# montekki/thaler-study

Hardware: AMD Instinct MI355X
Metric: field mul-adds/sec in sumcheck prover, n=28 vars (higher is better)
Workload: dtype u64

## Files before the change

### thaler-study_amd/csrc/kernels.hpp

```cpp
#pragma once
#include <hip/hip_runtime.h>

#include <type_traits>

#include "field.hpp"

namespace sc {

constexpr int kBlock = 256;
constexpr int kWave = 64;
constexpr int kMaxSums = 27;

typedef unsigned long long ull2 __attribute__((ext_vector_type(2)));

template <bool NT>
__device__ __forceinline__ ull2 ld16(const ull2* __restrict__ p) {
  if constexpr (NT) return __builtin_nontemporal_load(p);
  else return *p;
}
template <bool NT>
__device__ __forceinline__ void st16(ull2* __restrict__ p, ull2 v) {
  if constexpr (NT) __builtin_nontemporal_store(v, p);
  else *p = v;
}

struct FoldW {
  u64 w[16];
};

template <class F, int KF, int IN>
__device__ __forceinline__ void fold_run(const F& f, u64 (&v)[IN], const FoldW& fw) {
  if constexpr (KF == 1) {
    const u64 r0 = fw.w[1];
#pragma unroll
    for (int b = 0; b < IN / 2; ++b) v[b] = f.add(v[2 * b], f.mul(r0, f.sub(v[2 * b + 1], v[2 * b])));
  } else if constexpr (KF >= 2) {
    constexpr int G = 1 << KF;
#pragma unroll
    for (int b = 0; b < IN / G; ++b) {
      typename F::Acc3 acc;
      f.acc3_zero(acc);
#pragma unroll
      for (int c = 0; c < G; ++c) f.acc3_mac(acc, v[G * b + c], fw.w[c]);
      v[b] = f.acc3_get(acc);
    }
  }
}

template <class F>
__device__ __forceinline__ void extend_quads(const F& f, const X64 (&ta)[4], const X64 (&tb)[4], X64 (&ea)[3][3],
                                             X64 (&eb)[3][3]) {
  const X64 ha[4] = {ta[1], ta[3], ta[2], ta[3]}, la[4] = {ta[0], ta[2], ta[0], ta[1]};
  const X64 hb[4] = {tb[1], tb[3], tb[2], tb[3]}, lb[4] = {tb[0], tb[2], tb[0], tb[1]};
  X64 da[4], db[4];
  f.sub4(da, ha, la);
  f.sub4(db, hb, lb);
  const X64 ch[2] = {da[1], db[1]}, cl[2] = {da[0], db[0]};
  X64 corner[2];
  f.sub2(corner, ch, cl);
  ea[0][0] = ta[0]; ea[1][0] = ta[1]; ea[2][0] = da[0];
  ea[0][1] = ta[2]; ea[1][1] = ta[3]; ea[2][1] = da[1];
  ea[0][2] = da[2]; ea[1][2] = da[3]; ea[2][2] = corner[0];
  eb[0][0] = tb[0]; eb[1][0] = tb[1]; eb[2][0] = db[0];
  eb[0][1] = tb[2]; eb[1][1] = tb[3]; eb[2][1] = db[1];
  eb[0][2] = db[2]; eb[1][2] = db[3]; eb[2][2] = corner[1];
}

template <class F, int KS>
__device__ __forceinline__ void accumulate_run(const F& f, typename F::Acc* acc, const u64* a,
                                               const u64* b) {
  if constexpr (KS == 1) {
    f.acc_mac(acc[0], a[0], b[0]);
    f.acc_mac(acc[1], a[1], b[1]);
    f.acc_mac(acc[2], f.sub(a[1], a[0]), f.sub(b[1], b[0]));
  } else if constexpr (KS == 2) {
    X64 ea[3][3], eb[3][3];
    const X64 ta[4] = {split64(a[0]), split64(a[1]), split64(a[2]), split64(a[3])};
    const X64 tb[4] = {split64(b[0]), split64(b[1]), split64(b[2]), split64(b[3])};
    extend_quads(f, ta, tb, ea, eb);
#pragma unroll
    for (int u = 0; u < 3; ++u)
#pragma unroll
      for (int v = 0; v < 3; ++v) f.acc_mac(acc[3 * u + v], ea[u][v], eb[u][v]);
  }
}

template <class F>
__device__ __forceinline__ void accumulate_octet(const F& f, typename F::Acc* acc, const u64* a, const u64* b) {
#pragma unroll
  for (int step = 0; step < 3; ++step) {
    const int w = (step == 0) ? 0 : (step == 1) ? 2 : 1;
    X64 sa[4], sb[4];
    if (w == 2) {
      const X64 ah[4] = {split64(a[4]), split64(a[5]), split64(a[6]), split64(a[7])};
      const X64 al[4] = {split64(a[0]), split64(a[1]), split64(a[2]), split64(a[3])};
      const X64 bh[4] = {split64(b[4]), split64(b[5]), split64(b[6]), split64(b[7])};
      const X64 bl[4] = {split64(b[0]), split64(b[1]), split64(b[2]), split64(b[3])};
      f.sub4(sa, ah, al);
      f.sub4(sb, bh, bl);
    } else {
#pragma unroll
      for (int i = 0; i < 4; ++i) {
        sa[i] = split64(a[4 * w + i]);
        sb[i] = split64(b[4 * w + i]);
      }
    }
    X64 ea[3][3], eb[3][3];
    extend_quads(f, sa, sb, ea, eb);
#pragma unroll
    for (int u = 0; u < 3; ++u)
#pragma unroll
      for (int v = 0; v < 3; ++v) f.acc_mac(acc[(3 * u + v) * 3 + w], ea[u][v], eb[u][v]);
  }
}

__device__ __forceinline__ u64 shfl_down_u64(u64 v, int off) {
  return (u64)__shfl_down((unsigned long long)v, off, kWave);
}
__device__ __forceinline__ u64 shfl_u64(u64 v, int src) {
  return (u64)__shfl((unsigned long long)v, src, kWave);
}

template <class F, int NS>
__device__ __forceinline__ void block_reduce(const F& f, u64 (&res)[NS], u64* lds ) {
#pragma unroll
  for (int off = kWave / 2; off >= 1; off >>= 1) {
#pragma unroll
    for (int s = 0; s < NS; ++s) res[s] = f.add(res[s], shfl_down_u64(res[s], off));
  }
  const int lane = threadIdx.x & (kWave - 1), wave = threadIdx.x / kWave;
  if (lane == 0) {
#pragma unroll
    for (int s = 0; s < NS; ++s) lds[wave * NS + s] = res[s];
  }
  __syncthreads();
  if (threadIdx.x < NS) {
    u64 t = lds[threadIdx.x];
    const int n_waves = (int)blockDim.x / kWave;
    for (int w = 1; w < n_waves; ++w) t = f.add(t, lds[w * NS + threadIdx.x]);
    res[0] = t;
  }
}

__device__ __forceinline__ void write_split(u64* out, int s, u64 v) {
  out[2 * s] = v & 0xFFFFFFFFull;
  out[2 * s + 1] = v >> 32;
}

template <int NP>
__device__ __forceinline__ int swz_slot(int q) {
  if constexpr (NP == 1) return q;
  static_assert(NP == 2 || NP == 4 || NP == 8 || NP == 16, "pieces per lane");
  constexpr int SH = (NP == 2) ? 3 : (NP == 4) ? 2 : (NP == 8) ? 1 : 0;
  const int l = q / NP;
  return (q & ~(NP - 1)) | ((q ^ (l >> SH)) & (NP - 1));
}
__device__ __forceinline__ void wave_lds_sync() {
  asm volatile("s_waitcnt lgkmcnt(0)" ::: "memory");
  __builtin_amdgcn_wave_barrier();
}
template <int NP>
__device__ __forceinline__ void transpose_to_runs(ull2* __restrict__ lds, ull2 (&v)[NP], int lane) {
  if constexpr (NP > 1) {
#pragma unroll
    for (int k = 0; k < NP; ++k) lds[swz_slot<NP>(64 * k + lane)] = v[k];
    wave_lds_sync();
#pragma unroll
    for (int m = 0; m < NP; ++m) v[m] = lds[swz_slot<NP>(NP * lane + m)];
    wave_lds_sync();
  }
}
template <int NP>
__device__ __forceinline__ void transpose_to_pieces(ull2* __restrict__ lds, ull2 (&v)[NP], int lane) {
  if constexpr (NP > 1) {
#pragma unroll
    for (int m = 0; m < NP; ++m) lds[swz_slot<NP>(NP * lane + m)] = v[m];
    wave_lds_sync();
#pragma unroll
    for (int k = 0; k < NP; ++k) v[k] = lds[swz_slot<NP>(64 * k + lane)];
    wave_lds_sync();
  }
}

}

#include "kernels/pass.hpp"
#include "kernels/grid_pass.hpp"
#include "kernels/gram.hpp"
#include "kernels/mle.hpp"
#include "kernels/gkr.hpp"
#include "kernels/circuit.hpp"
#include "kernels/triangle.hpp"
#include "kernels/matmul.hpp"
#include "kernels/batch.hpp"
#include "kernels/sha256.hpp"
#include "kernels/merkle.hpp"
#include "kernels/pcs.hpp"
#include "kernels/row_code.hpp"
#include "kernels/ligero.hpp"
#include "kernels/ligero_long.hpp"
#include "kernels/rs_fold.hpp"
#include "kernels/expander.hpp"
#include "kernels/expander_long.hpp"
#include "kernels/peer.hpp"
#include "kernels/r1cs.hpp"
```

### thaler-study_amd/csrc/kernels/batch.hpp

```cpp
#pragma once

namespace sc {

constexpr int kBatchMaxBlocks = 128;
struct BatchDesc {
  const u64* a;
  const u64* b;
  u64* a2;
  u64* b2;
  GridW gw;
};
struct BatchOut {
  u64* partials;
  unsigned* tickets;
  u64* cells;
  u64* mailbox;
  u64 seq;
  int host_out;
};

template <class F, int KS>
__device__ __forceinline__ void batch_finish(const F& f, u64 total, const BatchOut& out, int inst) {
  constexpr int kPow3[6] = {1, 3, 9, 27, 81, 243};
  constexpr int cells = kPow3[KS], kLoads = 16;
  __shared__ int lds_flag;
  const int tid = threadIdx.x, n_blocks = gridDim.x;
  const u64* rows = out.partials + (size_t)inst * n_blocks * kGridChunk;
  if (tid < cells)
    __hip_atomic_store(out.partials + ((size_t)inst * n_blocks + blockIdx.x) * kGridChunk + tid, total, __ATOMIC_RELAXED,
                       __HIP_MEMORY_SCOPE_AGENT);
  asm volatile("s_waitcnt vmcnt(0)" ::: "memory");
  __syncthreads();
  if (tid == 0) {
    const unsigned t = __hip_atomic_fetch_add(out.tickets + 1 + inst, 1u, __ATOMIC_RELAXED, __HIP_MEMORY_SCOPE_AGENT);
    const int last = (t == (unsigned)n_blocks - 1) ? 1 : 0;
    if (last) {
      __builtin_amdgcn_fence(__ATOMIC_ACQUIRE, "agent");
      asm volatile("s_waitcnt vmcnt(0)" ::: "memory");
    }
    lds_flag = last;
  }
  __syncthreads();
  if (!lds_flag) return;
  if (tid < cells) {
    u64 s = 0;
    for (int q0 = 0; q0 < n_blocks; q0 += kLoads) {
      u64 x[kLoads];
#pragma unroll
      for (int q = 0; q < kLoads; ++q)
        x[q] = (q0 + q < n_blocks) ? __hip_atomic_load(rows + (size_t)(q0 + q) * kGridChunk + tid, __ATOMIC_RELAXED, __HIP_MEMORY_SCOPE_AGENT) : 0;
#pragma unroll
      for (int q = 0; q < kLoads; ++q) s = f.add(s, x[q]);
    }
    __hip_atomic_store(out.cells + (size_t)inst * kGridMaxCells + tid, s, __ATOMIC_RELAXED, __HIP_MEMORY_SCOPE_SYSTEM);
  }
  if (tid == 0) __hip_atomic_store(out.tickets + 1 + inst, 0u, __ATOMIC_RELAXED, __HIP_MEMORY_SCOPE_AGENT);
  asm volatile("s_waitcnt vmcnt(0)" ::: "memory");
  __syncthreads();
  if (tid == 0) {
    const unsigned t = __hip_atomic_fetch_add(out.tickets, 1u, __ATOMIC_RELAXED, __HIP_MEMORY_SCOPE_AGENT);
    if (t == gridDim.y - 1) {
      __builtin_amdgcn_fence(__ATOMIC_ACQUIRE, "agent");
      __hip_atomic_store(out.tickets, 0u, __ATOMIC_RELAXED, __HIP_MEMORY_SCOPE_AGENT);
      __hip_atomic_store(out.mailbox + kMailboxSeq, out.seq, __ATOMIC_RELEASE, __HIP_MEMORY_SCOPE_SYSTEM);
    }
  }
}

template <class F, int KS, bool PF>
__global__ void __launch_bounds__(kBlock)
batch_pass_kernel(F f, const BatchDesc* __restrict__ desc, int kf, size_t n_out, BatchOut out) {
  const int inst = blockIdx.y;
  const BatchDesc& d = desc[inst];
  const GridW gw = d.gw;
  const u64 total = wgrid_body<F, KS, PF>(f, d.a, d.b, d.a2, d.b2, gw, kf, n_out, out.host_out != 0);
  batch_finish<F, KS>(f, total, out, inst);
}

}
```

### thaler-study_amd/csrc/kernels/grid_pass.hpp

```cpp
#pragma once

namespace sc {

constexpr int kGridChunk = 256;
constexpr int kGridMaxVars = 5;
constexpr int kGridMaxCells = 243;
constexpr int kMailboxWide = 64;
constexpr int kMailboxWords = kMailboxWide + 512;
constexpr int kWgEntries = 32;
constexpr int kWgGroupBlocks = 32;
struct GridW {
  u64 w[1 << kGridMaxVars];
};
struct WgOut {
  u64* partials;
  u64* group_rows;
  unsigned* tickets;
  u64* mailbox;
  u64 seq;
  u64* limbs_dev;
  PeerX px;
  int host_out = 0;
};
template <class F, int KF>
__device__ __forceinline__ u64 grid_fold1(const F& f, const u64* __restrict__ T, u64* __restrict__ T2, const GridW& gw, size_t i, bool sys_out = false) {
  constexpr int FAN = 1 << KF, NPIECE = FAN / 2;
  const ull2* __restrict__ pt = reinterpret_cast<const ull2*>(T + i * FAN);
  ull2 x[NPIECE];
#pragma unroll
  for (int m = 0; m < NPIECE; ++m) x[m] = pt[m];
  typename F::Acc3 s;
  f.acc3_zero(s);
#pragma unroll
  for (int m = 0; m < NPIECE; ++m) {
    f.acc3_mac(s, x[m].x, gw.w[2 * m]);
    f.acc3_mac(s, x[m].y, gw.w[2 * m + 1]);
  }
  const u64 v = f.acc3_get(s);
  if (sys_out) __hip_atomic_store(T2 + i, v, __ATOMIC_RELAXED, __HIP_MEMORY_SCOPE_SYSTEM);
  else T2[i] = v;
  return v;
}
template <class F>
__global__ void __launch_bounds__(kBlock)
fold_wide_kernel(F f, const u64* __restrict__ T, u64* __restrict__ T2, GridW gw, int kf, size_t n_out) {
  for (size_t i = (size_t)blockIdx.x * kBlock + threadIdx.x; i < n_out; i += (size_t)gridDim.x * kBlock) {
    if (kf == 4) (void)grid_fold1<F, 4>(f, T, T2, gw, i);
    else (void)grid_fold1<F, 5>(f, T, T2, gw, i);
  }
}

template <class F, int KS, bool PF>
__device__ __forceinline__ u64 wgrid_body(const F& f, const u64* __restrict__ A, const u64* __restrict__ B, u64* __restrict__ A2,
                                          u64* __restrict__ B2, const GridW& gw, int kf, size_t n_out, bool sys_out) {
  constexpr int kWaves = kBlock / kWave;
  constexpr int kPow3[6] = {1, 3, 9, 27, 81, 243};
  constexpr int cells = kPow3[KS], G = 1 << KS, gpi = kWgEntries >> KS, pairs = gpi * cells;
  __shared__ u64 ext[kWaves][2][kGridChunk];
  __shared__ u64 red[kWaves][kGridChunk];
  __shared__ int cell_of[kWgEntries], suffix_of[kWgEntries];
  typedef __attribute__((address_space(3))) u64 lds_u64;
  const int tid = threadIdx.x, lane = tid & (kWave - 1), wave = tid / kWave;
  if (tid < kWgEntries) {
    int c = 0, u = 0, p3 = 1;
    for (int m = 0; m < KS; ++m) {
      c += ((tid >> (KS - 1 - m)) & 1) * p3;
      u += ((tid >> m) & 1) * p3;
      p3 *= 3;
    }
    cell_of[tid] = c;
    suffix_of[tid] = u;
  }
  __syncthreads();
  u64* const ef = &ext[wave][0][0];
  const int tbl = lane >> 5, ent = lane & (kWgEntries - 1);
  const int slot = tbl * kGridChunk + (ent >> KS) * cells + cell_of[ent & (G - 1)];
  const u64* __restrict__ src = tbl ? B : A;
  u64* __restrict__ dst = tbl ? B2 : A2;
  unsigned step[KS][3];
#pragma clang loop unroll(full)
  for (int j = 0; j < KS; ++j) {
    const int low = KS - 1 - j, pj = kPow3[j], stride = kPow3[low], items = (gpi * pj) << low;
    const unsigned inv = (1u << 20) / (unsigned)pj + 1u;
#pragma clang loop unroll(full)
    for (int q = 0; q < 3; ++q) {
      const int idx = lane + kWave * q;
      unsigned d = 0;
      if (idx < 2 * items) {
        const int tb = idx >= items ? 1 : 0, id = idx - tb * items;
        const int sfx = id & ((1 << low) - 1), t = id >> low;
        const int g = (int)(((unsigned)t * inv) >> 20), p = t - g * pj;
        d = 0x80000000u | (unsigned)(size_t)(lds_u64*)(ef + tb * kGridChunk + g * cells + p * 3 * stride + suffix_of[sfx]);
      }
      step[j][q] = d;
    }
  }
  typename F::Acc acc[4];
#pragma unroll
  for (int k = 0; k < 4; ++k) f.acc_zero(acc[k]);

  if constexpr (PF) {
    const size_t n_iter = (n_out + kWgEntries - 1) / kWgEntries;
    const size_t it0 = (size_t)blockIdx.x * kWaves + wave, it_stride = (size_t)gridDim.x * kWaves;
    ull2 nx0 = {0, 0}, nx1 = {0, 0};
    auto request = [&](size_t i) {
      if (kf == 0) {
        nx0.x = src[i];
      } else {
        const ull2* __restrict__ pt = reinterpret_cast<const ull2*>(src + i * 4);
        nx0 = pt[0];
        nx1 = pt[1];
      }
    };
    bool have = it0 < n_iter && it0 * kWgEntries + ent < n_out;
    if (have) request(it0 * kWgEntries + ent);
    for (size_t it = it0; it < n_iter; it += it_stride) {
      const size_t i = it * kWgEntries + ent;
      u64 v = 0;
      {
        const ull2 x0 = nx0, x1 = nx1;
        const bool mine = have;
        const size_t ni = (it + it_stride) * kWgEntries + ent;
        have = it + it_stride < n_iter && ni < n_out;
        if (have) request(ni);
        if (mine) {
          if (kf == 0) {
            v = x0.x;
          } else {
            typename F::Acc3 s;
            f.acc3_zero(s);
            f.acc3_mac(s, x0.x, gw.w[0]);
            f.acc3_mac(s, x0.y, gw.w[1]);
            f.acc3_mac(s, x1.x, gw.w[2]);
            f.acc3_mac(s, x1.y, gw.w[3]);
            v = f.acc3_get(s);
            if (sys_out) __hip_atomic_store(dst + i, v, __ATOMIC_RELAXED, __HIP_MEMORY_SCOPE_SYSTEM);
            else dst[i] = v;
          }
        }
      }
      ef[slot] = v;
      wave_lds_sync();
#pragma clang loop unroll(full)
      for (int j = 0; j < KS; ++j) {
        const int st = kPow3[KS - 1 - j];
#pragma clang loop unroll(full)
        for (int q = 0; q < 3; ++q) {
          if (2 * ((gpi * kPow3[j]) << (KS - 1 - j)) > kWave * q) {
            const unsigned d = step[j][q];
            if (d != 0) {
              lds_u64* const x = (lds_u64*)(size_t)(d & 0x7FFFFFFFu);
              x[2 * st] = f.sub(x[st], x[0]);
            }
          }
        }
        wave_lds_sync();
      }
#pragma unroll
      for (int k = 0; k < 4; ++k) {
        const int p = lane + kWave * k;
        if (p < pairs) f.acc_mac(acc[k], ef[p], ef[kGridChunk + p]);
      }
      wave_lds_sync();
    }
  } else {
    const size_t n_iter = (n_out + kWgEntries - 1) / kWgEntries;
    for (size_t it = (size_t)blockIdx.x * kWaves + wave; it < n_iter; it += (size_t)gridDim.x * kWaves) {
      const size_t i = it * kWgEntries + ent;
      u64 v = 0;
      if (i < n_out) {
        switch (kf) {
          case 0: v = src[i]; break;
          case 1: v = grid_fold1<F, 1>(f, src, dst, gw, i, sys_out); break;
          case 2: v = grid_fold1<F, 2>(f, src, dst, gw, i, sys_out); break;
          case 3: v = grid_fold1<F, 3>(f, src, dst, gw, i, sys_out); break;
          case 4: v = grid_fold1<F, 4>(f, src, dst, gw, i, sys_out); break;
          default: v = grid_fold1<F, 5>(f, src, dst, gw, i, sys_out); break;
        }
      }
      ef[slot] = v;
      wave_lds_sync();
#pragma clang loop unroll(full)
      for (int j = 0; j < KS; ++j) {
        const int st = kPow3[KS - 1 - j];
#pragma clang loop unroll(full)
        for (int q = 0; q < 3; ++q) {
          if (2 * ((gpi * kPow3[j]) << (KS - 1 - j)) > kWave * q) {
            const unsigned d = step[j][q];
            if (d != 0) {
              lds_u64* const x = (lds_u64*)(size_t)(d & 0x7FFFFFFFu);
              x[2 * st] = f.sub(x[st], x[0]);
            }
          }
        }
        wave_lds_sync();
      }
#pragma unroll
      for (int k = 0; k < 4; ++k) {
        const int p = lane + kWave * k;
        if (p < pairs) f.acc_mac(acc[k], ef[p], ef[kGridChunk + p]);
      }
      wave_lds_sync();
    }
  }

#pragma unroll
  for (int k = 0; k < 4; ++k) {
    const int p = lane + kWave * k;
    red[wave][p] = (p < pairs) ? f.acc_get(acc[k]) : 0;
  }
  __syncthreads();
  u64 total = 0;
  if (tid < cells) {
    for (int w = 0; w < kWaves; ++w)
      for (int g = 0; g < gpi; ++g) total = f.add(total, red[w][g * cells + tid]);
  }
  return total;
}

__device__ __forceinline__ void st16_system(u64* p, ull2 v) {
  asm volatile("global_store_dwordx4 %0, %1, off sc0 sc1" ::"v"(p), "v"(v) : "memory");
}
__device__ __forceinline__ ull2 ld16_system(const u64* p) {
  ull2 v;
  asm volatile("global_load_dwordx4 %0, %1, off sc0 sc1\n\ts_waitcnt vmcnt(0)" : "=v"(v) : "v"(p) : "memory");
  return v;
}
template <int CELLS>
__device__ __forceinline__ void exchange_wide(const WgOut& o, u64 total) {
  const PeerX& px = o.px;
  const int tid = threadIdx.x;
  const size_t par = (size_t)(px.tag & 1u) * kMaxPeers * kInboxWords;
  int err = 0;
  u64 lo = 0, hi = 0;
  if (tid < CELLS) {
    const size_t mine = par + (size_t)px.rank * kInboxWords + kInboxWide + 2 * (size_t)tid;
    const ull2 pair = {((u64)px.tag << 32) | (total & 0xFFFFFFFFull), ((u64)px.tag << 32) | (total >> 32)};
    for (int q = 0; q < px.world; ++q) st16_system(px.inbox[q] + mine, pair);
  }
  if (tid == CELLS) {
    const u64 g = ((u64)px.tag << 32) | (u64)px.digest;
    for (int q = 0; q < px.world; ++q)
      __hip_atomic_store(px.inbox[q] + par + (size_t)px.rank * kInboxWords + kInboxDigest, g, __ATOMIC_RELAXED, __HIP_MEMORY_SCOPE_SYSTEM);
  }
  const unsigned long long t0 = wall_clock64();
  if (tid < CELLS) {
    const u64* base = px.inbox[px.rank] + par + kInboxWide + 2 * (size_t)tid;
    for (int r = 0; r < px.world && !err; ++r) {
      unsigned spins = 0;
      while (true) {
        const ull2 g = ld16_system(base + (size_t)r * kInboxWords);
        if ((unsigned)(g.x >> 32) == px.tag && (unsigned)(g.y >> 32) == px.tag) {
          lo += g.x & 0xFFFFFFFFull;
          hi += g.y & 0xFFFFFFFFull;
          break;
        }
        if ((++spins & 31) == 0 && wall_clock64() - t0 > px.spin_ticks) {
          err = kXchgTimeout | (r << 8);
          break;
        }
        __builtin_amdgcn_s_sleep(1);
      }
    }
    st16_system(o.mailbox + kMailboxWide + 2 * tid, ull2{lo, hi});
  } else if (tid == CELLS) {
    const u64* base = px.inbox[px.rank] + par + kInboxDigest;
    for (int r = 0; r < px.world && !err; ++r) {
      unsigned spins = 0;
      while (true) {
        const u64 g = __hip_atomic_load(base + (size_t)r * kInboxWords, __ATOMIC_RELAXED, __HIP_MEMORY_SCOPE_SYSTEM);
        if ((unsigned)(g >> 32) == px.tag) {
          err = ((unsigned)g != px.digest) ? kXchgDigest : 0;
          break;
        }
        if ((++spins & 31) == 0 && wall_clock64() - t0 > px.spin_ticks) {
          err = kXchgTimeout | (r << 8);
          break;
        }
        __builtin_amdgcn_s_sleep(1);
      }
    }
  }
  __shared__ int worst;
  if (tid == 0) worst = 0;
  __syncthreads();
  if (err) atomicMax(&worst, err);
  asm volatile("s_waitcnt vmcnt(0)" ::: "memory");
  __syncthreads();
  if (tid == 0) {
    __hip_atomic_store(o.mailbox + kMailboxErr, (u64)worst, __ATOMIC_RELAXED, __HIP_MEMORY_SCOPE_SYSTEM);
    __hip_atomic_store(o.mailbox + kMailboxSeq, o.seq, __ATOMIC_RELEASE, __HIP_MEMORY_SCOPE_SYSTEM);
  }
}

template <int CELLS>
__device__ __forceinline__ void publish_cells(const WgOut& out, u64 total) {
  const int tid = threadIdx.x;
  if (out.px.world > 0) {
    exchange_wide<CELLS>(out, total);
    return;
  }
  if (out.limbs_dev) {
    if (tid < CELLS) write_split(out.limbs_dev, tid, total);
    return;
  }
  if (tid < CELLS) __hip_atomic_store(out.mailbox + kMailboxWide + tid, total, __ATOMIC_RELAXED, __HIP_MEMORY_SCOPE_SYSTEM);
  asm volatile("s_waitcnt vmcnt(0)" ::: "memory");
  __syncthreads();
  if (tid == 0) __hip_atomic_store(out.mailbox + kMailboxSeq, out.seq, __ATOMIC_RELEASE, __HIP_MEMORY_SCOPE_SYSTEM);
}

template <class F, int KS>
__device__ __forceinline__ void wgrid_finish(const F& f, u64 total, const WgOut& out) {
  constexpr int kPow3[6] = {1, 3, 9, 27, 81, 243};
  constexpr int cells = kPow3[KS];
  __shared__ int lds_flag;
  const int tid = threadIdx.x;
  if (gridDim.x > 1) {
    const int n_blocks = gridDim.x, group = blockIdx.x / kWgGroupBlocks, n_groups = (n_blocks + kWgGroupBlocks - 1) / kWgGroupBlocks;
    const int group_size = min(kWgGroupBlocks, n_blocks - group * kWgGroupBlocks);
    if (tid < cells)
      __hip_atomic_store(out.partials + (size_t)blockIdx.x * kGridChunk + tid, total, __ATOMIC_RELAXED, __HIP_MEMORY_SCOPE_AGENT);
    asm volatile("s_waitcnt vmcnt(0)" ::: "memory");
    __syncthreads();
    if (tid == 0) {
      const unsigned t = __hip_atomic_fetch_add(out.tickets + 1 + group, 1u, __ATOMIC_RELAXED, __HIP_MEMORY_SCOPE_AGENT);
      const int last = (t == (unsigned)group_size - 1) ? 1 : 0;
      if (last) {
        __builtin_amdgcn_fence(__ATOMIC_ACQUIRE, "agent");
        asm volatile("s_waitcnt vmcnt(0)" ::: "memory");
      }
      lds_flag = last;
    }
    __syncthreads();
    if (!lds_flag) return;
    total = 0;
    if (tid < cells) {
      u64 x[kWgGroupBlocks];
#pragma unroll
      for (int q = 0; q < kWgGroupBlocks; ++q)
        x[q] = (q < group_size) ? __hip_atomic_load(out.partials + (size_t)(group * kWgGroupBlocks + q) * kGridChunk + tid, __ATOMIC_RELAXED,
                                                    __HIP_MEMORY_SCOPE_AGENT)
                                : 0;
#pragma unroll
      for (int q = 0; q < kWgGroupBlocks; ++q) total = f.add(total, x[q]);
    }
    if (n_groups > 1) {
      __syncthreads();
      if (tid < cells)
        __hip_atomic_store(out.group_rows + (size_t)group * kGridChunk + tid, total, __ATOMIC_RELAXED, __HIP_MEMORY_SCOPE_AGENT);
      asm volatile("s_waitcnt vmcnt(0)" ::: "memory");
      __syncthreads();
      if (tid == 0) {
        const unsigned t = __hip_atomic_fetch_add(out.tickets, 1u, __ATOMIC_RELAXED, __HIP_MEMORY_SCOPE_AGENT);
        const int last = (t == (unsigned)n_groups - 1) ? 1 : 0;
        if (last) {
          __builtin_amdgcn_fence(__ATOMIC_ACQUIRE, "agent");
          asm volatile("s_waitcnt vmcnt(0)" ::: "memory");
        }
        lds_flag = last;
      }
      __syncthreads();
      if (!lds_flag) return;
      total = 0;
      if (tid < cells) {
        u64 x[kWgGroupBlocks];
#pragma unroll
        for (int q = 0; q < kWgGroupBlocks; ++q)
          x[q] = (q < n_groups) ? __hip_atomic_load(out.group_rows + (size_t)q * kGridChunk + tid, __ATOMIC_RELAXED, __HIP_MEMORY_SCOPE_AGENT) : 0;
#pragma unroll
        for (int q = 0; q < kWgGroupBlocks; ++q) total = f.add(total, x[q]);
      }
    }
    if (tid <= n_groups) __hip_atomic_store(out.tickets + tid, 0u, __ATOMIC_RELAXED, __HIP_MEMORY_SCOPE_AGENT);
  }
  publish_cells<cells>(out, total);
}

template <class F, int KS, bool PF>
__global__ void __launch_bounds__(kBlock)
wgrid_pass_kernel(F f, const u64* __restrict__ A, const u64* __restrict__ B, u64* __restrict__ A2, u64* __restrict__ B2,
                  GridW gw, int kf, size_t n_out, WgOut out) {
  const u64 total = wgrid_body<F, KS, PF>(f, A, B, A2, B2, gw, kf, n_out, out.host_out != 0);
  wgrid_finish<F, KS>(f, total, out);
}

constexpr int kWfThreads = 512;
template <class F, int KF, int KS, bool NT>
__global__ void __launch_bounds__(kWfThreads)
wfold_pass_kernel(F f, const u64* __restrict__ A, const u64* __restrict__ B, u64* __restrict__ A2, u64* __restrict__ B2, FoldW fw,
                  u64 r_top, size_t n_tiles, WgOut out) {
  static_assert(KF == 4 || KF == 5, "four or five pending challenges");
  static_assert(KS >= 1 && KS <= 5, "one to five rounds");
  constexpr int OUT = 4, NPS = 8, NP = 32;
  constexpr int OUTS = kWave >> (KF - 4);
  constexpr int TILE_OUT = OUT * OUTS;
  constexpr int NPO = TILE_OUT / (2 * kWave);
  constexpr int kWaves = kWfThreads / kWave;
  constexpr int kPow3[6] = {1, 3, 9, 27, 81, 243};
  constexpr int cells = kPow3[KS], G = 1 << KS, gpi = kWgEntries >> KS, pairs = gpi * cells;
  constexpr int kRegionWords = 1024 + 512 + 512;
  __shared__ u64 lds_all[kWaves * kRegionWords];
  __shared__ int cell_of[kWgEntries], suffix_of[kWgEntries];
  __shared__ unsigned lds_next;
  typedef __attribute__((address_space(3))) u64 lds_u64;
  const int tid = threadIdx.x, lane = tid & (kWave - 1), wave = tid / kWave;
  if (tid < kWgEntries) {
    int c = 0, u = 0, p3 = 1;
    for (int m = 0; m < KS; ++m) {
      c += ((tid >> (KS - 1 - m)) & 1) * p3;
      u += ((tid >> m) & 1) * p3;
      p3 *= 3;
    }
    cell_of[tid] = c;
    suffix_of[tid] = u;
  }
  if (tid == 0) lds_next = 0;
  __syncthreads();
  ull2* const reg = reinterpret_cast<ull2*>(lds_all + (size_t)wave * kRegionWords);
  u64* const xchg = lds_all + (size_t)wave * kRegionWords + 1024;
  u64* const ef = xchg + 512;
  const int tbl = lane >> 5, ent = lane & (kWgEntries - 1);
  const int slot = tbl * kGridChunk + (ent >> KS) * cells + cell_of[ent & (G - 1)];
  unsigned step[KS][3];
#pragma clang loop unroll(full)
  for (int j = 0; j < KS; ++j) {
    const int low = KS - 1 - j, pj = kPow3[j], stride = kPow3[low], items = (gpi * pj) << low;
    const unsigned inv = (1u << 20) / (unsigned)pj + 1u;
#pragma clang loop unroll(full)
    for (int q = 0; q < 3; ++q) {
      const int idx = lane + kWave * q;
      unsigned d = 0;
      if (idx < 2 * items) {
        const int tb = idx >= items ? 1 : 0, id = idx - tb * items;
        const int sfx = id & ((1 << low) - 1), t = id >> low;
        const int g = (int)(((unsigned)t * inv) >> 20), pp = t - g * pj;
        d = 0x80000000u | (unsigned)(size_t)(lds_u64*)(ef + tb * kGridChunk + g * cells + pp * 3 * stride + suffix_of[sfx]);
      }
      step[j][q] = d;
    }
  }
  typename F::Acc acc[4];
#pragma unroll
  for (int k = 0; k < 4; ++k) f.acc_zero(acc[k]);

  const ull2* __restrict__ Ap = reinterpret_cast<const ull2*>(A);
  const ull2* __restrict__ Bp = reinterpret_cast<const ull2*>(B);
  ull2* __restrict__ A2p = reinterpret_cast<ull2*>(A2);
  ull2* __restrict__ B2p = reinterpret_cast<ull2*>(B2);
  const int rot = wave & 3;
  auto next_tile = [&]() -> size_t {
    unsigned c = 0;
    if (lane == 0) c = __hip_atomic_fetch_add(&lds_next, 1u, __ATOMIC_RELAXED, __HIP_MEMORY_SCOPE_WORKGROUP);
    return (size_t)__builtin_amdgcn_readfirstlane(c) * gridDim.x + blockIdx.x;
  };
  auto load_sub = [&](const ull2* __restrict__ T, size_t tile, int o, ull2 (&p)[NPS]) {
    const ull2* src = T + tile * kWave * NP + (size_t)o * NPS * kWave + lane;
#pragma unroll
    for (int k = 0; k < NPS; ++k) p[k] = ld16<NT>(src + k * kWave);
  };
  auto stash = [&](const ull2 (&p)[NPS]) {
#pragma unroll
    for (int k = 0; k < NPS; ++k) reg[swz_slot<NPS>(64 * k + lane)] = p[k];
  };
  auto fold16 = [&]() -> u64 {
    typename F::Acc3 sacc;
    f.acc3_zero(sacc);
#pragma unroll
    for (int m = 0; m < NPS; ++m) {
      const ull2 x = reg[swz_slot<NPS>(NPS * lane + m)];
      f.acc3_mac(sacc, x.x, fw.w[2 * m]);
      f.acc3_mac(sacc, x.y, fw.w[2 * m + 1]);
    }
    const u64 h = f.acc3_get(sacc);
    if constexpr (KF == 5) {
      const u64 hn = __shfl_xor(h, 1);
      return f.add(h, f.mul(r_top, f.sub(hn, h)));
    } else {
      return h;
    }
  };
  auto put = [&](u64* dst, int o, u64 x) {
    if constexpr (KF == 5) {
      if ((lane & 1) == 0) dst[OUTS * o + (lane >> 1)] = x;
    } else {
      dst[OUTS * o + lane] = x;
    }
  };
  auto grid_group = [&](int grp) {
    ef[slot] = xchg[kWave * OUT * tbl + kWgEntries * grp + ent];
    wave_lds_sync();
#pragma clang loop unroll(full)
    for (int j = 0; j < KS; ++j) {
      const int st = kPow3[KS - 1 - j];
#pragma clang loop unroll(full)
      for (int q = 0; q < 3; ++q) {
        if (2 * ((gpi * kPow3[j]) << (KS - 1 - j)) > kWave * q) {
          const unsigned d = step[j][q];
          if (d != 0) {
            lds_u64* const x = (lds_u64*)(size_t)(d & 0x7FFFFFFFu);
            x[2 * st] = f.sub(x[st], x[0]);
          }
        }
      }
      wave_lds_sync();
    }
#pragma unroll
    for (int k = 0; k < 4; ++k) {
      const int p = lane + kWave * k;
      if (p < pairs) f.acc_mac(acc[k], ef[p], ef[kGridChunk + p]);
    }
    wave_lds_sync();
  };
  ull2 pa[NPS], pb[NPS];
  size_t tile = next_tile();
  if (tile < n_tiles) {
    load_sub(Ap, tile, rot, pa);
    load_sub(Bp, tile, rot, pb);
  }
  while (tile < n_tiles) {
    const size_t next = next_tile();
#pragma unroll
    for (int i = 0; i < OUT; ++i) {
      const int o = (i + rot) & 3, no = (i + 1 + rot) & 3;
      stash(pa);
      wave_lds_sync();
      if (i + 1 < OUT) load_sub(Ap, tile, no, pa);
      else if (next < n_tiles) load_sub(Ap, next, no, pa);
      const u64 xa = fold16();
      wave_lds_sync();
      stash(pb);
      wave_lds_sync();
      if (i + 1 < OUT) load_sub(Bp, tile, no, pb);
      else if (next < n_tiles) load_sub(Bp, next, no, pb);
      const u64 xb = fold16();
      put(xchg, o, xa);
      put(xchg + kWave * OUT, o, xb);
      wave_lds_sync();
#pragma unroll 1
      for (int g = 0; g < OUTS / kWgEntries; ++g) grid_group(o * (OUTS / kWgEntries) + g);
    }
    {
      const ull2* xo = reinterpret_cast<const ull2*>(xchg);
      const size_t o0 = tile * kWave * NPO;
#pragma unroll
      for (int k = 0; k < NPO; ++k) {
        const size_t q = o0 + (size_t)k * kWave + lane;
        st16<false>(A2p + q, xo[kWave * k + lane]);
        st16<false>(B2p + q, xo[kWave * OUT / 2 + kWave * k + lane]);
      }
    }
    wave_lds_sync();
    if (wave == 0 && blockIdx.x < 8) asm volatile("buffer_wbl2 sc1" ::: "memory");
    tile = next;
  }
  __syncthreads();
  u64* const red = lds_all;
#pragma unroll
  for (int k = 0; k < 4; ++k) {
    const int p = lane + kWave * k;
    red[wave * kGridChunk + p] = (p < pairs) ? f.acc_get(acc[k]) : 0;
  }
  __syncthreads();
  u64 total = 0;
  if (tid < cells) {
    for (int w = 0; w < kWaves; ++w)
      for (int g = 0; g < gpi; ++g) total = f.add(total, red[w * kGridChunk + g * cells + tid]);
  }
  wgrid_finish<F, KS>(f, total, out);
}

template <class F>
__global__ void __launch_bounds__(kBlock)
rank_pass_kernel(F f, const u64* __restrict__ A, const u64* __restrict__ B, u64* __restrict__ A2, u64* __restrict__ B2, GridW gw, int kf,
                 WgOut out) {
  const PeerX& px = out.px;
  __shared__ u64 ta[kMaxPeers], tb[kMaxPeers];
  __shared__ int worst;
  const int tid = threadIdx.x;
  const size_t par = (size_t)(px.tag & 1u) * kMaxPeers * kInboxWords;
  int err = 0;
  if (tid == 0) worst = 0;
  if (tid < 2) {
    const u64* __restrict__ src = tid ? B : A;
    const int fan = 1 << kf;
    u64 v = 0;
    for (int c = 0; c < fan; ++c) v = f.add(v, f.mul(src[c], gw.w[c]));
    const ull2 pair = {((u64)px.tag << 32) | (v & 0xFFFFFFFFull), ((u64)px.tag << 32) | (v >> 32)};
    const size_t mine = par + (size_t)px.rank * kInboxWords + kInboxWide + 2 * (size_t)tid;
    for (int q = 0; q < px.world; ++q) st16_system(px.inbox[q] + mine, pair);
  }
  if (tid == 2) {
    const u64 g = ((u64)px.tag << 32) | (u64)px.digest;
    for (int q = 0; q < px.world; ++q)
      __hip_atomic_store(px.inbox[q] + par + (size_t)px.rank * kInboxWords + kInboxDigest, g, __ATOMIC_RELAXED, __HIP_MEMORY_SCOPE_SYSTEM);
  }
  const unsigned long long t0 = wall_clock64();
  if (tid < 3 * px.world) {
    const int r = tid / 3, what = tid % 3;
    const u64* base = px.inbox[px.rank] + par + (size_t)r * kInboxWords;
    unsigned spins = 0;
    while (true) {
      if (what < 2) {
        const ull2 g = ld16_system(base + kInboxWide + 2 * what);
        if ((unsigned)(g.x >> 32) == px.tag && (unsigned)(g.y >> 32) == px.tag) {
          const u64 v = (g.x & 0xFFFFFFFFull) | (g.y << 32);
          (what ? tb : ta)[r] = v;
          break;
        }
      } else {
        const u64 g = __hip_atomic_load(base + kInboxDigest, __ATOMIC_RELAXED, __HIP_MEMORY_SCOPE_SYSTEM);
        if ((unsigned)(g >> 32) == px.tag) {
          err = ((unsigned)g != px.digest) ? kXchgDigest : 0;
          break;
        }
      }
      if ((++spins & 31) == 0 && wall_clock64() - t0 > px.spin_ticks) {
        err = kXchgTimeout | (r << 8);
        break;
      }
      __builtin_amdgcn_s_sleep(1);
    }
  }
  __syncthreads();
  if (err) atomicMax(&worst, err);
  __syncthreads();
  if (worst == 0) {
    if (tid < px.world) {
      A2[tid] = ta[tid];
      B2[tid] = tb[tid];
    }
    int g = 0;
    while ((1 << g) < px.world) ++g;
    int cells = 1;
    for (int j = 0; j < g; ++j) cells *= 3;
    if (tid < cells) {
      int d[3] = {0, 0, 0};
      int c = tid;
      for (int j = g - 1; j >= 0; --j) {
        d[j] = c % 3;
        c /= 3;
      }
      u64 ea = 0, eb = 0;
      for (int e = 0; e < px.world; ++e) {
        int sign = 1;
        for (int j = 0; j < g; ++j) {
          const int b = (e >> j) & 1;
          if (d[j] == 2) sign = b ? sign : -sign;
          else if (d[j] != b) sign = 0;
        }
        if (sign > 0) {
          ea = f.add(ea, ta[e]);
          eb = f.add(eb, tb[e]);
        } else if (sign < 0) {
          ea = f.sub(ea, ta[e]);
          eb = f.sub(eb, tb[e]);
        }
      }
      __hip_atomic_store(out.mailbox + kMailboxWide + tid, f.mul(ea, eb), __ATOMIC_RELAXED, __HIP_MEMORY_SCOPE_SYSTEM);
    }
  }
  asm volatile("s_waitcnt vmcnt(0)" ::: "memory");
  __syncthreads();
  if (tid == 0) {
    __hip_atomic_store(out.mailbox + kMailboxErr, (u64)worst, __ATOMIC_RELAXED, __HIP_MEMORY_SCOPE_SYSTEM);
    __hip_atomic_store(out.mailbox + kMailboxSeq, out.seq, __ATOMIC_RELEASE, __HIP_MEMORY_SCOPE_SYSTEM);
  }
}

}
```

Measured before the change: 875.7 billion.

## Issue first tile loads before LDS table setup and prefetch next fold in wgrid

Moves the first global loads of each wave ahead of the shared-memory table initialization and block barrier, so memory latency overlaps setup. The dynamic tile counter now starts at kWaves, with each wave statically taking its first tile. Adds an AHEAD path for Goldilocks Montgomery that folds the next iteration's entries after the current accumulation, and raises launch bounds to request 4 blocks per CU. This risks more register pressure from the kGridMaxPieces staging array, and the launch-bounds hint may cause spills.

```diff
diff --git a/thaler-study_amd/csrc/kernels.hpp b/thaler-study_amd/csrc/kernels.hpp
--- a/thaler-study_amd/csrc/kernels.hpp
+++ b/thaler-study_amd/csrc/kernels.hpp
@@ -158,6 +158,11 @@
 __device__ __forceinline__ void wave_lds_sync() {
   asm volatile("s_waitcnt lgkmcnt(0)" ::: "memory");
   __builtin_amdgcn_wave_barrier();
+}
+__device__ __forceinline__ void block_lds_sync() {
+  asm volatile("s_waitcnt lgkmcnt(0)" ::: "memory");
+  __builtin_amdgcn_s_barrier();
+  asm volatile("" ::: "memory");
 }
 template <int NP>
 __device__ __forceinline__ void transpose_to_runs(ull2* __restrict__ lds, ull2 (&v)[NP], int lane) {
diff --git a/thaler-study_amd/csrc/kernels/batch.hpp b/thaler-study_amd/csrc/kernels/batch.hpp
--- a/thaler-study_amd/csrc/kernels/batch.hpp
+++ b/thaler-study_amd/csrc/kernels/batch.hpp
@@ -73,7 +73,7 @@
   const int inst = blockIdx.y;
   const BatchDesc& d = desc[inst];
   const GridW gw = d.gw;
-  const u64 total = wgrid_body<F, KS, PF>(f, d.a, d.b, d.a2, d.b2, gw, kf, n_out, out.host_out != 0);
+  const u64 total = wgrid_body<F, KS, PF, false>(f, d.a, d.b, d.a2, d.b2, gw, kf, n_out, out.host_out != 0);
   batch_finish<F, KS>(f, total, out, inst);
 }
 
diff --git a/thaler-study_amd/csrc/kernels/grid_pass.hpp b/thaler-study_amd/csrc/kernels/grid_pass.hpp
--- a/thaler-study_amd/csrc/kernels/grid_pass.hpp
+++ b/thaler-study_amd/csrc/kernels/grid_pass.hpp
@@ -22,13 +22,17 @@
   PeerX px;
   int host_out = 0;
 };
-template <class F, int KF>
-__device__ __forceinline__ u64 grid_fold1(const F& f, const u64* __restrict__ T, u64* __restrict__ T2, const GridW& gw, size_t i, bool sys_out = false) {
+constexpr int kGridMaxPieces = (1 << kGridMaxVars) / 2;
+template <int KF>
+__device__ __forceinline__ void grid_load1(const u64* __restrict__ T, size_t i, ull2 (&x)[kGridMaxPieces]) {
   constexpr int FAN = 1 << KF, NPIECE = FAN / 2;
   const ull2* __restrict__ pt = reinterpret_cast<const ull2*>(T + i * FAN);
-  ull2 x[NPIECE];
 #pragma unroll
   for (int m = 0; m < NPIECE; ++m) x[m] = pt[m];
+}
+template <class F, int KF>
+__device__ __forceinline__ u64 grid_sum1(const F& f, const ull2 (&x)[kGridMaxPieces], u64* __restrict__ T2, const GridW& gw, size_t i, bool sys_out) {
+  constexpr int FAN = 1 << KF, NPIECE = FAN / 2;
   typename F::Acc3 s;
   f.acc3_zero(s);
 #pragma unroll
@@ -40,6 +44,12 @@
   if (sys_out) __hip_atomic_store(T2 + i, v, __ATOMIC_RELAXED, __HIP_MEMORY_SCOPE_SYSTEM);
   else T2[i] = v;
   return v;
+}
+template <class F, int KF>
+__device__ __forceinline__ u64 grid_fold1(const F& f, const u64* __restrict__ T, u64* __restrict__ T2, const GridW& gw, size_t i, bool sys_out = false) {
+  ull2 x[kGridMaxPieces];
+  grid_load1<KF>(T, i, x);
+  return grid_sum1<F, KF>(f, x, T2, gw, i, sys_out);
 }
 template <class F>
 __global__ void __launch_bounds__(kBlock)
@@ -50,7 +60,16 @@
   }
 }
 
-template <class F, int KS, bool PF>
+__device__ __forceinline__ void wgrid_request(const u64* __restrict__ src, size_t i, int kf, ull2& nx0, ull2& nx1) {
+  if (kf == 0) {
+    nx0.x = src[i];
+  } else {
+    const ull2* __restrict__ pt = reinterpret_cast<const ull2*>(src + i * 4);
+    nx0 = pt[0];
+    nx1 = pt[1];
+  }
+}
+template <class F, int KS, bool PF, bool AHEAD = std::is_same<F, GoldilocksMont>::value>
 __device__ __forceinline__ u64 wgrid_body(const F& f, const u64* __restrict__ A, const u64* __restrict__ B, u64* __restrict__ A2,
                                           u64* __restrict__ B2, const GridW& gw, int kf, size_t n_out, bool sys_out) {
   constexpr int kWaves = kBlock / kWave;
@@ -61,6 +80,28 @@
   __shared__ int cell_of[kWgEntries], suffix_of[kWgEntries];
   typedef __attribute__((address_space(3))) u64 lds_u64;
   const int tid = threadIdx.x, lane = tid & (kWave - 1), wave = tid / kWave;
+  [[maybe_unused]] ull2 nx0 = {0, 0}, nx1 = {0, 0};
+  [[maybe_unused]] ull2 x0[kGridMaxPieces];
+  [[maybe_unused]] bool have = false;
+  if constexpr (PF || AHEAD) {
+    const u64* __restrict__ src0 = (lane >> 5) ? B : A;
+    const size_t it0 = (size_t)blockIdx.x * kWaves + wave, i = it0 * kWgEntries + (lane & (kWgEntries - 1));
+    have = it0 < (n_out + kWgEntries - 1) / kWgEntries && i < n_out;
+    if (have) {
+      if constexpr (PF) {
+        wgrid_request(src0, i, kf, nx0, nx1);
+      } else {
+        switch (kf) {
+          case 0: x0[0].x = src0[i]; break;
+          case 1: grid_load1<1>(src0, i, x0); break;
+          case 2: grid_load1<2>(src0, i, x0); break;
+          case 3: grid_load1<3>(src0, i, x0); break;
+          case 4: grid_load1<4>(src0, i, x0); break;
+          default: grid_load1<5>(src0, i, x0); break;
+        }
+      }
+    }
+  }
   if (tid < kWgEntries) {
     int c = 0, u = 0, p3 = 1;
     for (int m = 0; m < KS; ++m) {
@@ -71,7 +112,7 @@
     cell_of[tid] = c;
     suffix_of[tid] = u;
   }
-  __syncthreads();
+  block_lds_sync();
   u64* const ef = &ext[wave][0][0];
   const int tbl = lane >> 5, ent = lane & (kWgEntries - 1);
   const int slot = tbl * kGridChunk + (ent >> KS) * cells + cell_of[ent & (G - 1)];
@@ -102,18 +143,6 @@
   if constexpr (PF) {
     const size_t n_iter = (n_out + kWgEntries - 1) / kWgEntries;
     const size_t it0 = (size_t)blockIdx.x * kWaves + wave, it_stride = (size_t)gridDim.x * kWaves;
-    ull2 nx0 = {0, 0}, nx1 = {0, 0};
-    auto request = [&](size_t i) {
-      if (kf == 0) {
-        nx0.x = src[i];
-      } else {
-        const ull2* __restrict__ pt = reinterpret_cast<const ull2*>(src + i * 4);
-        nx0 = pt[0];
-        nx1 = pt[1];
-      }
-    };
-    bool have = it0 < n_iter && it0 * kWgEntries + ent < n_out;
-    if (have) request(it0 * kWgEntries + ent);
     for (size_t it = it0; it < n_iter; it += it_stride) {
       const size_t i = it * kWgEntries + ent;
       u64 v = 0;
@@ -122,7 +151,7 @@
         const bool mine = have;
         const size_t ni = (it + it_stride) * kWgEntries + ent;
         have = it + it_stride < n_iter && ni < n_out;
-        if (have) request(ni);
+        if (have) wgrid_request(src, ni, kf, nx0, nx1);
         if (mine) {
           if (kf == 0) {
             v = x0.x;
@@ -162,6 +191,58 @@
         if (p < pairs) f.acc_mac(acc[k], ef[p], ef[kGridChunk + p]);
       }
       wave_lds_sync();
+    }
+  } else if constexpr (AHEAD) {
+    const size_t n_iter = (n_out + kWgEntries - 1) / kWgEntries;
+    const size_t it0 = (size_t)blockIdx.x * kWaves + wave, it_stride = (size_t)gridDim.x * kWaves;
+    u64 v = 0;
+    if (have) {
+      const size_t i = it0 * kWgEntries + ent;
+      switch (kf) {
+        case 0: v = x0[0].x; break;
+        case 1: v = grid_sum1<F, 1>(f, x0, dst, gw, i, sys_out); break;
+        case 2: v = grid_sum1<F, 2>(f, x0, dst, gw, i, sys_out); break;
+        case 3: v = grid_sum1<F, 3>(f, x0, dst, gw, i, sys_out); break;
+        case 4: v = grid_sum1<F, 4>(f, x0, dst, gw, i, sys_out); break;
+        default: v = grid_sum1<F, 5>(f, x0, dst, gw, i, sys_out); break;
+      }
+    }
+    for (size_t it = it0; it < n_iter; it += it_stride) {
+      ef[slot] = v;
+      wave_lds_sync();
+#pragma clang loop unroll(full)
+      for (int j = 0; j < KS; ++j) {
+        const int st = kPow3[KS - 1 - j];
+#pragma clang loop unroll(full)
+        for (int q = 0; q < 3; ++q) {
+          if (2 * ((gpi * kPow3[j]) << (KS - 1 - j)) > kWave * q) {
+            const unsigned d = step[j][q];
+            if (d != 0) {
+              lds_u64* const x = (lds_u64*)(size_t)(d & 0x7FFFFFFFu);
+              x[2 * st] = f.sub(x[st], x[0]);
+            }
+          }
+        }
+        wave_lds_sync();
+      }
+#pragma unroll
+      for (int k = 0; k < 4; ++k) {
+        const int p = lane + kWave * k;
+        if (p < pairs) f.acc_mac(acc[k], ef[p], ef[kGridChunk + p]);
+      }
+      wave_lds_sync();
+      const size_t i = (it + it_stride) * kWgEntries + ent;
+      v = 0;
+      if (it + it_stride < n_iter && i < n_out) {
+        switch (kf) {
+          case 0: v = src[i]; break;
+          case 1: v = grid_fold1<F, 1>(f, src, dst, gw, i, sys_out); break;
+          case 2: v = grid_fold1<F, 2>(f, src, dst, gw, i, sys_out); break;
+          case 3: v = grid_fold1<F, 3>(f, src, dst, gw, i, sys_out); break;
+          case 4: v = grid_fold1<F, 4>(f, src, dst, gw, i, sys_out); break;
+          default: v = grid_fold1<F, 5>(f, src, dst, gw, i, sys_out); break;
+        }
+      }
     }
   } else {
     const size_t n_iter = (n_out + kWgEntries - 1) / kWgEntries;
@@ -378,7 +459,7 @@
 }
 
 template <class F, int KS, bool PF>
-__global__ void __launch_bounds__(kBlock)
+__global__ void __launch_bounds__(kBlock, 4)
 wgrid_pass_kernel(F f, const u64* __restrict__ A, const u64* __restrict__ B, u64* __restrict__ A2, u64* __restrict__ B2,
                   GridW gw, int kf, size_t n_out, WgOut out) {
   const u64 total = wgrid_body<F, KS, PF>(f, A, B, A2, B2, gw, kf, n_out, out.host_out != 0);
@@ -405,6 +486,20 @@
   __shared__ unsigned lds_next;
   typedef __attribute__((address_space(3))) u64 lds_u64;
   const int tid = threadIdx.x, lane = tid & (kWave - 1), wave = tid / kWave;
+  const ull2* __restrict__ Ap = reinterpret_cast<const ull2*>(A);
+  const ull2* __restrict__ Bp = reinterpret_cast<const ull2*>(B);
+  const int rot = wave & 3;
+  auto load_sub = [&](const ull2* __restrict__ T, size_t tile, int o, ull2 (&p)[NPS]) {
+    const ull2* src = T + tile * kWave * NP + (size_t)o * NPS * kWave + lane;
+#pragma unroll
+    for (int k = 0; k < NPS; ++k) p[k] = ld16<NT>(src + k * kWave);
+  };
+  ull2 pa[NPS], pb[NPS];
+  size_t tile = (size_t)wave * gridDim.x + blockIdx.x;
+  if (tile < n_tiles) {
+    load_sub(Ap, tile, rot, pa);
+    load_sub(Bp, tile, rot, pb);
+  }
   if (tid < kWgEntries) {
     int c = 0, u = 0, p3 = 1;
     for (int m = 0; m < KS; ++m) {
@@ -415,8 +510,8 @@
     cell_of[tid] = c;
     suffix_of[tid] = u;
   }
-  if (tid == 0) lds_next = 0;
-  __syncthreads();
+  if (tid == 0) lds_next = kWaves;
+  block_lds_sync();
   ull2* const reg = reinterpret_cast<ull2*>(lds_all + (size_t)wave * kRegionWords);
   u64* const xchg = lds_all + (size_t)wave * kRegionWords + 1024;
   u64* const ef = xchg + 512;
@@ -444,20 +539,12 @@
 #pragma unroll
   for (int k = 0; k < 4; ++k) f.acc_zero(acc[k]);
 
-  const ull2* __restrict__ Ap = reinterpret_cast<const ull2*>(A);
-  const ull2* __restrict__ Bp = reinterpret_cast<const ull2*>(B);
   ull2* __restrict__ A2p = reinterpret_cast<ull2*>(A2);
   ull2* __restrict__ B2p = reinterpret_cast<ull2*>(B2);
-  const int rot = wave & 3;
   auto next_tile = [&]() -> size_t {
     unsigned c = 0;
     if (lane == 0) c = __hip_atomic_fetch_add(&lds_next, 1u, __ATOMIC_RELAXED, __HIP_MEMORY_SCOPE_WORKGROUP);
     return (size_t)__builtin_amdgcn_readfirstlane(c) * gridDim.x + blockIdx.x;
-  };
-  auto load_sub = [&](const ull2* __restrict__ T, size_t tile, int o, ull2 (&p)[NPS]) {
-    const ull2* src = T + tile * kWave * NP + (size_t)o * NPS * kWave + lane;
-#pragma unroll
-    for (int k = 0; k < NPS; ++k) p[k] = ld16<NT>(src + k * kWave);
   };
   auto stash = [&](const ull2 (&p)[NPS]) {
 #pragma unroll
@@ -512,12 +599,6 @@
     }
     wave_lds_sync();
   };
-  ull2 pa[NPS], pb[NPS];
-  size_t tile = next_tile();
-  if (tile < n_tiles) {
-    load_sub(Ap, tile, rot, pa);
-    load_sub(Bp, tile, rot, pb);
-  }
   while (tile < n_tiles) {
     const size_t next = next_tile();
 #pragma unroll
```

Measured after the change: 877.4 billion, median of 3. No clear change (+0.2%).
